# mederrata/spmf

Measured on AMD Instinct MI355X. Metric: elbo_steps_per_sec, higher is better.
Workload: dtype f32

## Files before the change

### spmf_amd/csrc/widek.hip

```cpp
#include "common.h"
#include "kernels.h"

namespace spmf {

namespace {

constexpr int kInFlight = 4;

__device__ __forceinline__ float4 ld4(const float* __restrict__ base, int row, int KP, int sub) {
  return *reinterpret_cast<const float4*>(base + (size_t)row * KP + sub * 4);
}
template <int NH>
__device__ __forceinline__ float group_dot(float4 a, float4 b) {
  if constexpr (NH == 2) {
    const float v = group_sum<16>(dot4(a, b));
    return v + __shfl_xor(v, 16);
  } else {
    return wave_sum(fmaf(a.w, b.w, fmaf(a.z, b.z, fmaf(a.y, b.y, fmaf(a.x, b.x, 0.f)))));
  }
}
template <int NH>
__device__ __forceinline__ float xhalf_add(float v) {
  if constexpr (NH == 2) v += __shfl_xor(v, 32);
  return v;
}
template <int NH>
__device__ __forceinline__ float4 xhalf_add(float4 v) {
  return make_float4(xhalf_add<NH>(v.x), xhalf_add<NH>(v.y), xhalf_add<NH>(v.z), xhalf_add<NH>(v.w));
}

}

template <int KP>
__global__ __launch_bounds__(256) void row_widek_kernel(
    int64_t B, const int32_t* __restrict__ row_ptr, const int32_t* __restrict__ col,
    const float* __restrict__ val, const float* __restrict__ row_scale, const float* __restrict__ Ap,
    const float* __restrict__ Vp, const float* __restrict__ phi, const double* __restrict__ dprep,
    float* __restrict__ z, float* __restrict__ gzs, double* __restrict__ dacc, int mode, int Dcols,
    int64_t dacc_stride) {
  constexpr int NH = 256 / KP, LPG = 64 / NH;
  if (gridDim.y > 1) {
    const size_t sd = blockIdx.y;
    Ap += sd * (size_t)Dcols * KP;
    Vp += sd * (size_t)Dcols * KP;
    phi += sd * (size_t)Dcols;
    dprep += sd * (size_t)kPrepSeg * (KP + 1);
    z += sd * (size_t)B * KP;
    gzs += sd * (size_t)B * KP;
    dacc += sd * (size_t)dacc_stride;
  }
  const bool encode_only = mode == 1;
  const int lane = threadIdx.x & 63, sub = lane % LPG, h = lane / LPG;
  const int64_t wave = ((int64_t)blockIdx.x * blockDim.x + threadIdx.x) >> 6;
  const int64_t nwaves = ((int64_t)gridDim.x * blockDim.x) >> 6;
  float4 veta = make_float4(0.f, 0.f, 0.f, 0.f);
  if (!encode_only)
    veta = make_float4((float)prep_sum(dprep, KP, sub * 4 + 0), (float)prep_sum(dprep, KP, sub * 4 + 1),
                       (float)prep_sum(dprep, KP, sub * 4 + 2), (float)prep_sum(dprep, KP, sub * 4 + 3));
  double ll_acc = 0.0, zsq_acc = 0.0, nnf_acc = 0.0;
  float4 zsum = make_float4(0.f, 0.f, 0.f, 0.f);
  for (int64_t b = wave; b < B; b += nwaves) {
    const int start = row_ptr[b], end = row_ptr[b + 1];
    const float xi = row_scale ? row_scale[b] : 1.f;
    float4 zacc = make_float4(0.f, 0.f, 0.f, 0.f);
    for (int base = start; base < end; base += 64) {
      const int i = base + lane;
      const int c = i < end ? col[i] : 0;
      const float x = i < end ? val[i] : 0.f;
      const int cnt = min(64, end - base);
      for (int e0 = 0; e0 < cnt; e0 += NH * kInFlight) {
        float4 a[kInFlight];
        float xe[kInFlight];
#pragma unroll
        for (int j = 0; j < kInFlight; ++j) {
          const int idx = e0 + NH * j + h, src = min(idx, 63);
          const int cj = __shfl(c, src);
          const float xs = (NH == 2 || idx < cnt) ? __shfl(x, src) : 0.f;
          xe[j] = idx < cnt ? xs : 0.f;
          a[j] = ld4(Ap, cj, KP, sub);
        }
#pragma unroll
        for (int j = 0; j < kInFlight; ++j) zacc = fma4(xe[j], a[j], zacc);
      }
    }
    zacc = xhalf_add<NH>(zacc);
    zacc.x *= xi; zacc.y *= xi; zacc.z *= xi; zacc.w *= xi;
    if (h == 0) reinterpret_cast<float4*>(z + (size_t)b * KP)[sub] = zacc;
    if (encode_only) continue;
    float4 gz = make_float4(0.f, 0.f, 0.f, 0.f);
    float llrow = 0.f;
    for (int base = start; base < end; base += 64) {
      const int i = base + lane;
      const int c = i < end ? col[i] : 0;
      const float x = i < end ? val[i] : 0.f;
      const int cnt = min(64, end - base);
      for (int e0 = 0; e0 < cnt; e0 += NH * kInFlight) {
        float4 vv[kInFlight];
        float xe[kInFlight], ph[kInFlight];
#pragma unroll
        for (int j = 0; j < kInFlight; ++j) {
          const int idx = e0 + NH * j + h, src = min(idx, 63);
          const int cj = __shfl(c, src);
          const float xs = (NH == 2 || idx < cnt) ? __shfl(x, src) : 0.f;
          xe[j] = idx < cnt ? xs : 0.f;
          vv[j] = ld4(Vp, cj, KP, sub);
          ph[j] = phi[cj];
        }
#pragma unroll
        for (int j = 0; j < kInFlight; ++j) {
          const float r = group_dot<NH>(zacc, vv[j]) + ph[j];
          const bool on = xe[j] > 0.f, good = r > 0.f && r < INFINITY;
          const float cc = on ? (good ? xe[j] * __builtin_amdgcn_rcpf(r) : 1.f) : 0.f;
          if (on && good) llrow = fmaf(xe[j], logf(r), llrow);
          if (on && !good) nnf_acc += 1.0;
          gz = fma4(cc, vv[j], gz);
        }
      }
    }
    gz = xhalf_add<NH>(gz);
    if (h == 0) {
      float4 o;
      o.x = xi * (gz.x - veta.x - zacc.x);
      o.y = xi * (gz.y - veta.y - zacc.y);
      o.z = xi * (gz.z - veta.z - zacc.z);
      o.w = xi * (gz.w - veta.w - zacc.w);
      reinterpret_cast<float4*>(gzs + (size_t)b * KP)[sub] = o;
      if constexpr (NH == 2) {
        zsq_acc += (double)dot4(zacc, zacc);
      } else {
        zsq_acc += (double)(zacc.x * zacc.x);
        zsq_acc += (double)(zacc.y * zacc.y);
        zsq_acc += (double)(zacc.z * zacc.z);
        zsq_acc += (double)(zacc.w * zacc.w);
      }
      zsum = add4(zsum, zacc);
    }
    ll_acc += (double)llrow;
  }
  if (encode_only) return;
  dacc += (size_t)(blockIdx.x % kDaccRep) * (kDaccHead + KP);
  const double zq = wave_sum(zsq_acc);
  if (sub == 0) {
    atomicAdd(&dacc[0], ll_acc);
    if (nnf_acc != 0.0) atomicAdd(&dacc[2], nnf_acc);
  }
  if (lane == 0) atomicAdd(&dacc[1], zq);
  if (h == 0) {
    atomicAdd(&dacc[kDaccHead + sub * 4 + 0], (double)zsum.x);
    atomicAdd(&dacc[kDaccHead + sub * 4 + 1], (double)zsum.y);
    atomicAdd(&dacc[kDaccHead + sub * 4 + 2], (double)zsum.z);
    atomicAdd(&dacc[kDaccHead + sub * 4 + 3], (double)zsum.w);
  }
}

template <int KP>
__global__ __launch_bounds__(256) void col_widek_kernel(
    int D, int n_panels, int row_base, int blocks_per_panel, const int32_t* __restrict__ item_ptr,
    const int4* __restrict__ items, const int32_t* __restrict__ pc_row, const float* __restrict__ pc_val,
    const float* __restrict__ Vp, const float* __restrict__ phi, const float* __restrict__ z,
    const float* __restrict__ gzs, float* __restrict__ gAp, float* __restrict__ gVp, float* __restrict__ gphi,
    const int32_t* __restrict__ item_mid, int half_sel, int64_t Brows, int64_t acc_stride,
    const double* __restrict__ pack_dacc, float* __restrict__ pack_tail, int64_t dacc_stride) {
  constexpr int NH = 256 / KP, LPG = 64 / NH;
  if (pack_dacc && blockIdx.x == 0) {
    const double* dacc = pack_dacc + (size_t)blockIdx.y * dacc_stride;
    float* tail = pack_tail + (size_t)blockIdx.y * acc_stride;
    for (int i = threadIdx.x; i < kDaccHead + KP; i += blockDim.x) fold_dacc(i, dacc, tail, KP);
    return;
  }
  if (gridDim.y > 1) {
    const size_t sd = blockIdx.y;
    Vp += sd * (size_t)D * KP;
    phi += sd * (size_t)D;
    z += sd * (size_t)Brows * KP;
    gzs += sd * (size_t)Brows * KP;
    gAp += sd * (size_t)acc_stride;
    gVp += sd * (size_t)acc_stride;
    gphi += sd * (size_t)acc_stride;
  }
  const int lane = threadIdx.x & 63, wid = threadIdx.x >> 6, sub = lane % LPG, h = lane / LPG;
  const int64_t L = (int64_t)blockIdx.x - (pack_dacc ? 1 : 0);
  const int p = (int)(L / blocks_per_panel), ib = (int)(L % blocks_per_panel);
  if (p >= n_panels) return;
  const int ilo = half_sel == 2 ? item_mid[p] : item_ptr[p];
  const int ihi = half_sel == 1 ? item_mid[p] : item_ptr[p + 1];
  const int it = ilo + ib * 4 + wid;
  if (it >= ihi) return;
  const int4 im = items[it];
  const int d = im.z;
  const float4 vp = ld4(Vp, d, KP, sub);
  const float ph = phi[d];
  float4 gV = make_float4(0.f, 0.f, 0.f, 0.f), gA = gV;
  float gph = 0.f;
  const int end = im.x + im.y;
  for (int base = im.x; base < end; base += 64) {
    const int i = base + lane;
    const int rb = i < end ? pc_row[i] - row_base : 0;
    const float x = i < end ? pc_val[i] : 0.f;
    const int cnt = min(64, end - base);
    for (int e0 = 0; e0 < cnt; e0 += NH * kInFlight) {
      float4 zz[kInFlight], gg[kInFlight];
      float xe[kInFlight];
#pragma unroll
      for (int j = 0; j < kInFlight; ++j) {
        const int idx = e0 + NH * j + h, src = min(idx, 63);
        const int b = __shfl(rb, src);
        const float xs = (NH == 2 || idx < cnt) ? __shfl(x, src) : 0.f;
        xe[j] = idx < cnt ? xs : 0.f;
        zz[j] = ld4(z, b, KP, sub);
        gg[j] = ld4(gzs, b, KP, sub);
      }
#pragma unroll
      for (int j = 0; j < kInFlight; ++j) {
        const float r = group_dot<NH>(zz[j], vp) + ph;
        const float xr = (r > 0.f && r < INFINITY) ? xe[j] * __builtin_amdgcn_rcpf(r) : (xe[j] > 0.f ? 1.f : 0.f);
        gV = fma4(xr, zz[j], gV);
        gA = fma4(xe[j], gg[j], gA);
        gph += xr;
      }
    }
  }
  gV = xhalf_add<NH>(gV);
  gA = xhalf_add<NH>(gA);
  gph = xhalf_add<NH>(gph);
  if (h == 0) {
    float* dv = gVp + (size_t)d * KP + sub * 4;
    float* da = gAp + (size_t)d * KP + sub * 4;
    if (gV.x != 0.f) atomicAdd(dv + 0, gV.x);
    if (gV.y != 0.f) atomicAdd(dv + 1, gV.y);
    if (gV.z != 0.f) atomicAdd(dv + 2, gV.z);
    if (gV.w != 0.f) atomicAdd(dv + 3, gV.w);
    if (gA.x != 0.f) atomicAdd(da + 0, gA.x);
    if (gA.y != 0.f) atomicAdd(da + 1, gA.y);
    if (gA.z != 0.f) atomicAdd(da + 2, gA.z);
    if (gA.w != 0.f) atomicAdd(da + 3, gA.w);
    if (lane == 0 && gph != 0.f) atomicAdd(&gphi[d], gph);
  }
}

namespace {
template <int KP>
void row_widek(int nb, const RowArgs& a, hipStream_t st) {
  hipLaunchKernelGGL((row_widek_kernel<KP>), dim3(nb, a.S > 1 ? a.S : 1), dim3(256), 0, st, a.B, a.row_ptr, a.col,
                     a.val, a.row_scale, a.Ap, a.Vp, a.phi, a.dprep, a.z, a.gzs, a.dacc, a.mode, a.D,
                     a.dacc_stride);
}
template <int KP>
void col_widek(int64_t nb, int bpp, const ColArgs& a, hipStream_t st) {
  hipLaunchKernelGGL((col_widek_kernel<KP>), dim3((unsigned)nb, a.S > 1 ? a.S : 1), dim3(256), 0, st, a.D,
                     a.n_panels, a.row_base, bpp, a.item_ptr, reinterpret_cast<const int4*>(a.items), a.pc_row,
                     a.pc_val, a.Vp, a.phi, a.z, a.gzs, a.gAp, a.gVp, a.gphi, a.item_mid, a.half_sel, a.B,
                     a.acc_stride, a.pack_dacc, a.pack_tail, a.dacc_stride);
}
}

bool launch_row_widek(int KP, const RowArgs& a, hipStream_t st) {
  if (a.logt != 0 || (a.mode != 0 && a.mode != 1) || a.det_slots) return false;
  const int64_t want = (a.B + 3) / 4;
  const int nb = (int)(want < 1 ? 1 : (want > 2048 ? 2048 : want));
  return with_kp<256, 128>(KP, [&](auto kp) { row_widek<decltype(kp)::value>(nb, a, st); });
}

bool launch_col_widek(int KP, const ColArgs& a, hipStream_t st) {
  if (a.logt != 0 || a.det_part) return false;
  const int bpp = (a.max_items_per_panel + 3) / 4;
  if (bpp < 1) return false;
  const int64_t nb = (int64_t)a.n_panels * bpp + (a.pack_dacc ? 1 : 0);
  return with_kp<256, 128>(KP, [&](auto kp) { col_widek<decltype(kp)::value>(nb, bpp, a, st); });
}

}
```

Baseline: 379.7.

## Rework wide-K row/col kernels with prefetch, DPP reductions, packed entries, dynamic tail

Rewrites both wide-K kernels. Gather depth grows to groups of 8, and per-entry group dot products are replaced with a three-step DPP/swizzle transpose-fold that reduces eight dots at once. Row pointers and entry chunks are prefetched one and two rows ahead, and a work-stealing dynamic tail balances uneven rows. Optional packed 16+16-bit entries shrink index traffic. The col kernel interleaves panel mapping across blocks and combines halves through LDS before the atomics. This adds complexity and depends on new args (ent, dyn_tail, panel_rows, dyn slot) defined elsewhere. Packed mode truncates values to integers up to 65535.

```diff
diff --git a/spmf_amd/csrc/widek.hip b/spmf_amd/csrc/widek.hip
--- a/spmf_amd/csrc/widek.hip
+++ b/spmf_amd/csrc/widek.hip
@@ -5,40 +5,184 @@
 
 namespace {
 
-constexpr int kInFlight = 4;
+constexpr int kGroup = 8;
+constexpr int kRowBlocks = 2048;
+constexpr int kDynNum = 1, kDynDen = 8;
 
 __device__ __forceinline__ float4 ld4(const float* __restrict__ base, int row, int KP, int sub) {
   return *reinterpret_cast<const float4*>(base + (size_t)row * KP + sub * 4);
 }
+__device__ __forceinline__ float4 zero4() { return make_float4(0.f, 0.f, 0.f, 0.f); }
+
+template <int M>
+__device__ __forceinline__ float lane_xor(float v) {
+  if constexpr (M == 1) {
+    return __int_as_float(__builtin_amdgcn_update_dpp(0, __float_as_int(v), 0xB1, 0xF, 0xF, true));
+  } else if constexpr (M == 2) {
+    return __int_as_float(__builtin_amdgcn_update_dpp(0, __float_as_int(v), 0x4E, 0xF, 0xF, true));
+  } else if constexpr (M < 32) {
+    return __int_as_float(__builtin_amdgcn_ds_swizzle(__float_as_int(v), (M << 10) | 0x1f));
+  } else {
+    return __shfl_xor(v, 32);
+  }
+}
+__host__ __device__ constexpr int fold8_entry(int l) { return ((l & 1) << 2) | (l & 2) | ((l >> 2) & 1); }
+template <int LPG>
+__device__ __forceinline__ float fold8(const float (&p)[kGroup], int lane) {
+  static_assert(kGroup == 8, "three halving steps");
+  const bool b0 = lane & 1, b1 = lane & 2, b2 = lane & 4;
+  float q[4], r[2];
+#pragma unroll
+  for (int i = 0; i < 4; ++i) q[i] = (b0 ? p[i + 4] : p[i]) + lane_xor<1>(b0 ? p[i] : p[i + 4]);
+#pragma unroll
+  for (int i = 0; i < 2; ++i) r[i] = (b1 ? q[i + 2] : q[i]) + lane_xor<2>(b1 ? q[i] : q[i + 2]);
+  float v = (b2 ? r[1] : r[0]) + lane_xor<4>(b2 ? r[0] : r[1]);
+  v += lane_xor<8>(v);
+  v += lane_xor<16>(v);
+  if constexpr (LPG == 64) v += lane_xor<32>(v);
+  return v;
+}
 template <int NH>
-__device__ __forceinline__ float group_dot(float4 a, float4 b) {
+__device__ __forceinline__ int bcast_i(int v, int idx, int h) {
+  const int lo = __builtin_amdgcn_readlane(v, idx);
   if constexpr (NH == 2) {
-    const float v = group_sum<16>(dot4(a, b));
-    return v + __shfl_xor(v, 16);
-  } else {
-    return wave_sum(fmaf(a.w, b.w, fmaf(a.z, b.z, fmaf(a.y, b.y, fmaf(a.x, b.x, 0.f)))));
-  }
+    const int hi = __builtin_amdgcn_readlane(v, idx + 1);
+    return h ? hi : lo;
+  }
+  return lo;
 }
 template <int NH>
-__device__ __forceinline__ float xhalf_add(float v) {
-  if constexpr (NH == 2) v += __shfl_xor(v, 32);
-  return v;
+__device__ __forceinline__ float bcast_f(float v, int idx, int h) {
+  return __int_as_float(bcast_i<NH>(__float_as_int(v), idx, h));
+}
+template <int NH>
+__device__ __forceinline__ float owner_bcast(float w, int j, int h) {
+  const int lo = __builtin_amdgcn_readlane(__float_as_int(w), fold8_entry(j));
+  if constexpr (NH == 2) {
+    const int hi = __builtin_amdgcn_readlane(__float_as_int(w), 32 + fold8_entry(j));
+    return __int_as_float(h ? hi : lo);
+  }
+  return __int_as_float(lo);
 }
 template <int NH>
 __device__ __forceinline__ float4 xhalf_add(float4 v) {
-  return make_float4(xhalf_add<NH>(v.x), xhalf_add<NH>(v.y), xhalf_add<NH>(v.z), xhalf_add<NH>(v.w));
-}
-
-}
-
-template <int KP>
+  if constexpr (NH == 2) {
+    v.x += __shfl_xor(v.x, 32); v.y += __shfl_xor(v.y, 32);
+    v.z += __shfl_xor(v.z, 32); v.w += __shfl_xor(v.w, 32);
+  }
+  return v;
+}
+
+template <bool PACKED>
+__device__ __forceinline__ void ld_entry(const int32_t* __restrict__ idx, const float* __restrict__ val,
+                                         const uint32_t* __restrict__ ent, int i, bool ok, int& ra, float& rb) {
+  if constexpr (PACKED) {
+    ra = ok ? (int)ent[i] : 0;
+    rb = 0.f;
+  } else {
+    ra = ok ? idx[i] : 0;
+    rb = ok ? val[i] : 0.f;
+  }
+}
+template <bool PACKED>
+__device__ __forceinline__ void entry_of(int ra, float rb, int& c, float& x) {
+  if constexpr (PACKED) {
+    c = (int)((uint32_t)ra >> 16);
+    x = (float)((uint32_t)ra & 0xffffu);
+  } else {
+    c = ra;
+    x = rb;
+  }
+}
+
+template <int KP, bool FULL>
+__device__ __forceinline__ void row_s1_group(const float* __restrict__ Ap, int c, float x, int e0, int cnt, int sub,
+                                             int h, float4& zacc) {
+  constexpr int NH = 256 / KP;
+  float4 a[kGroup];
+  float xe[kGroup];
+#pragma unroll
+  for (int j = 0; j < kGroup; ++j) {
+    const int i0 = e0 + NH * j;
+    const int cj = bcast_i<NH>(c, i0, h);
+    xe[j] = bcast_f<NH>(x, i0, h);
+    a[j] = (FULL || i0 + h < cnt) ? ld4(Ap, cj, KP, sub) : zero4();
+  }
+#pragma unroll
+  for (int j = 0; j < kGroup; ++j) zacc = fma4(xe[j], a[j], zacc);
+}
+template <int KP, bool FULL>
+__device__ __forceinline__ void row_s2_group(const float* __restrict__ Vp, const float* __restrict__ phi, int c,
+                                             float x, int e0, int cnt, int lane, int sub, int h, const float4& z,
+                                             float4& gz, float& ll, double& nnf) {
+  constexpr int NH = 256 / KP, LPG = 64 / NH;
+  float4 vv[kGroup];
+#pragma unroll
+  for (int j = 0; j < kGroup; ++j) {
+    const int i0 = e0 + NH * j;
+    const int cj = bcast_i<NH>(c, i0, h);
+    vv[j] = (FULL || i0 + h < cnt) ? ld4(Vp, cj, KP, sub) : zero4();
+  }
+  const int mine = e0 + NH * fold8_entry(lane & 7) + h;
+  const int cs = __shfl(c, mine);
+  const float xs = __shfl(x, mine);
+  const float ph = phi[cs];
+  float p[kGroup];
+#pragma unroll
+  for (int j = 0; j < kGroup; ++j) p[j] = dot4(z, vv[j]);
+  const float r = fold8<LPG>(p, lane) + ph;
+  const bool on = mine < cnt && xs > 0.f, good = r > 0.f && r < INFINITY;
+  const float cc = on ? (good ? xs * __builtin_amdgcn_rcpf(r) : 1.f) : 0.f;
+  if (sub < 8) {
+    ll = fmaf(on && good ? xs : 0.f, logf(good ? r : 1.f), ll);
+    if (on && !good) nnf += 1.0;
+  }
+#pragma unroll
+  for (int j = 0; j < kGroup; ++j) gz = fma4(owner_bcast<NH>(cc, j, h), vv[j], gz);
+}
+
+template <int KP, bool FULL>
+__device__ __forceinline__ void col_group(const float* __restrict__ z, const float* __restrict__ gzs, int rb, float x,
+                                          int e0, int cnt, int lane, int sub, int h, const float4& vp, float ph,
+                                          float4& gV, float4& gA, float& gph) {
+  constexpr int NH = 256 / KP, LPG = 64 / NH;
+  float4 zz[kGroup], gg[kGroup];
+  float xe[kGroup];
+#pragma unroll
+  for (int j = 0; j < kGroup; ++j) {
+    const int i0 = e0 + NH * j;
+    const int b = bcast_i<NH>(rb, i0, h);
+    xe[j] = bcast_f<NH>(x, i0, h);
+    const bool ld = FULL || i0 + h < cnt;
+    zz[j] = ld ? ld4(z, b, KP, sub) : zero4();
+    gg[j] = ld ? ld4(gzs, b, KP, sub) : zero4();
+  }
+  const int mine = e0 + NH * fold8_entry(lane & 7) + h;
+  const float xs = __shfl(x, mine);
+  float p[kGroup];
+#pragma unroll
+  for (int j = 0; j < kGroup; ++j) p[j] = dot4(zz[j], vp);
+  const float r = fold8<LPG>(p, lane) + ph;
+  const float xr = (r > 0.f && r < INFINITY) ? xs * __builtin_amdgcn_rcpf(r) : (xs > 0.f ? 1.f : 0.f);
+  if (sub < 8) gph += xr;
+#pragma unroll
+  for (int j = 0; j < kGroup; ++j) {
+    gV = fma4(owner_bcast<NH>(xr, j, h), zz[j], gV);
+    gA = fma4(xe[j], gg[j], gA);
+  }
+}
+
+}
+
+template <int KP, bool PACKED>
 __global__ __launch_bounds__(256) void row_widek_kernel(
     int64_t B, const int32_t* __restrict__ row_ptr, const int32_t* __restrict__ col,
-    const float* __restrict__ val, const float* __restrict__ row_scale, const float* __restrict__ Ap,
-    const float* __restrict__ Vp, const float* __restrict__ phi, const double* __restrict__ dprep,
-    float* __restrict__ z, float* __restrict__ gzs, double* __restrict__ dacc, int mode, int Dcols,
-    int64_t dacc_stride) {
+    const float* __restrict__ val, const uint32_t* __restrict__ ent, const float* __restrict__ row_scale,
+    const float* __restrict__ Ap, const float* __restrict__ Vp, const float* __restrict__ phi,
+    const double* __restrict__ dprep, float* __restrict__ z, float* __restrict__ gzs, double* __restrict__ dacc,
+    int mode, int Dcols, int64_t dacc_stride, int dyn_tail) {
   constexpr int NH = 256 / KP, LPG = 64 / NH;
+  constexpr int EG = NH * kGroup;
   if (gridDim.y > 1) {
     const size_t sd = blockIdx.y;
     Ap += sd * (size_t)Dcols * KP;
@@ -51,100 +195,148 @@
   }
   const bool encode_only = mode == 1;
   const int lane = threadIdx.x & 63, sub = lane % LPG, h = lane / LPG;
-  const int64_t wave = ((int64_t)blockIdx.x * blockDim.x + threadIdx.x) >> 6;
+  const int64_t wave = (int64_t)blockIdx.x * (blockDim.x >> 6) +
+                       __builtin_amdgcn_readfirstlane((int)(threadIdx.x >> 6));
   const int64_t nwaves = ((int64_t)gridDim.x * blockDim.x) >> 6;
-  float4 veta = make_float4(0.f, 0.f, 0.f, 0.f);
+  float4 veta = zero4();
   if (!encode_only)
     veta = make_float4((float)prep_sum(dprep, KP, sub * 4 + 0), (float)prep_sum(dprep, KP, sub * 4 + 1),
                        (float)prep_sum(dprep, KP, sub * 4 + 2), (float)prep_sum(dprep, KP, sub * 4 + 3));
   double ll_acc = 0.0, zsq_acc = 0.0, nnf_acc = 0.0;
-  float4 zsum = make_float4(0.f, 0.f, 0.f, 0.f);
-  for (int64_t b = wave; b < B; b += nwaves) {
-    const int start = row_ptr[b], end = row_ptr[b + 1];
-    const float xi = row_scale ? row_scale[b] : 1.f;
-    float4 zacc = make_float4(0.f, 0.f, 0.f, 0.f);
-    for (int base = start; base < end; base += 64) {
-      const int i = base + lane;
-      const int c = i < end ? col[i] : 0;
-      const float x = i < end ? val[i] : 0.f;
-      const int cnt = min(64, end - base);
-      for (int e0 = 0; e0 < cnt; e0 += NH * kInFlight) {
-        float4 a[kInFlight];
-        float xe[kInFlight];
-#pragma unroll
-        for (int j = 0; j < kInFlight; ++j) {
-          const int idx = e0 + NH * j + h, src = min(idx, 63);
-          const int cj = __shfl(c, src);
-          const float xs = (NH == 2 || idx < cnt) ? __shfl(x, src) : 0.f;
-          xe[j] = idx < cnt ? xs : 0.f;
-          a[j] = ld4(Ap, cj, KP, sub);
-        }
-#pragma unroll
-        for (int j = 0; j < kInFlight; ++j) zacc = fma4(xe[j], a[j], zacc);
+  float4 zsum = zero4();
+
+  int64_t B_static = B, dyn_lo = B, dyn_hi = B;
+  unsigned int* dyn_ctr = nullptr;
+  if (dyn_tail && !encode_only) {
+    const int64_t per_wave = B / nwaves;
+    if (per_wave >= 8) {
+      int64_t fixed = per_wave - (per_wave * kDynNum) / kDynDen;
+      if (fixed < 2) fixed = 2;
+      B_static = fixed * nwaves;
+      const int r = (int)(wave & (kDaccRep - 1));
+      const int64_t each = (B - B_static + kDaccRep - 1) / kDaccRep;
+      dyn_lo = B_static + r * each;
+      dyn_hi = dyn_lo + each < B ? dyn_lo + each : B;
+      if (dyn_lo > B) dyn_lo = B;
+      dyn_ctr = reinterpret_cast<unsigned int*>(dacc + (size_t)r * (kDaccHead + KP) + kDaccDynSlot);
+    }
+  }
+  auto fixed_next = [&](int64_t cur) -> int64_t {
+    if (cur >= B) return B;
+    if (cur + nwaves < B_static) return cur + nwaves;
+    return dyn_ctr ? (int64_t)-1 : B;
+  };
+  auto take_dynamic = [&]() -> int64_t {
+    unsigned int k = 0;
+    if (lane == 0) k = atomicAdd(dyn_ctr, 1u);
+    k = (unsigned int)__builtin_amdgcn_readfirstlane((int)k);
+    const int64_t row = dyn_lo + (int64_t)k;
+    return row < dyn_hi ? row : B;
+  };
+  auto ptr_of = [&](int64_t row, int& s, int& e, float& sc) {
+    s = __builtin_amdgcn_readfirstlane(row_ptr[row]);
+    e = __builtin_amdgcn_readfirstlane(row_ptr[row + 1]);
+    sc = row_scale ? row_scale[row] : 1.f;
+  };
+
+  int start = 0, end = 0, pc = 0, nstart = 0, nend = 0;
+  float xi = 1.f, px = 0.f, nxi = 1.f;
+  int64_t b = wave < B_static ? wave : B;
+  int64_t bn = fixed_next(b);
+  if (bn < 0) bn = take_dynamic();
+  int64_t bnn = fixed_next(bn);
+  if (bnn < 0) bnn = take_dynamic();
+  if (b < B) {
+    ptr_of(b, start, end, xi);
+    ld_entry<PACKED>(col, val, ent, start + lane, start + lane < end, pc, px);
+  }
+  if (bn < B) ptr_of(bn, nstart, nend, nxi);
+  while (b < B) {
+    int qc = 0, nnstart = 0, nnend = 0;
+    float qx = 0.f, nnxi = 1.f;
+    if (bn < B) ld_entry<PACKED>(col, val, ent, nstart + lane, nstart + lane < nend, qc, qx);
+    if (bnn < B) ptr_of(bnn, nnstart, nnend, nnxi);
+    int64_t bnnn = fixed_next(bnn);
+    unsigned int dyn_k = 0;
+    const bool dyn_ask = bnnn < 0;
+    if (dyn_ask && lane == 0) dyn_k = atomicAdd(dyn_ctr, 1u);
+    float4 zacc = zero4();
+    {
+      int ra = pc;
+      float rb = px;
+      for (int base = start; base < end; base += 64) {
+        int ra2;
+        float rb2;
+        const int i2 = base + 64 + lane;
+        ld_entry<PACKED>(col, val, ent, i2, i2 < end, ra2, rb2);
+        int c;
+        float x;
+        entry_of<PACKED>(ra, rb, c, x);
+        const int cnt = min(64, end - base);
+        int e0 = 0;
+        for (; e0 + EG <= cnt; e0 += EG) row_s1_group<KP, true>(Ap, c, x, e0, cnt, sub, h, zacc);
+        if (e0 < cnt) row_s1_group<KP, false>(Ap, c, x, e0, cnt, sub, h, zacc);
+        ra = ra2;
+        rb = rb2;
       }
     }
     zacc = xhalf_add<NH>(zacc);
     zacc.x *= xi; zacc.y *= xi; zacc.z *= xi; zacc.w *= xi;
     if (h == 0) reinterpret_cast<float4*>(z + (size_t)b * KP)[sub] = zacc;
-    if (encode_only) continue;
-    float4 gz = make_float4(0.f, 0.f, 0.f, 0.f);
+    float4 gz = zero4();
     float llrow = 0.f;
-    for (int base = start; base < end; base += 64) {
-      const int i = base + lane;
-      const int c = i < end ? col[i] : 0;
-      const float x = i < end ? val[i] : 0.f;
-      const int cnt = min(64, end - base);
-      for (int e0 = 0; e0 < cnt; e0 += NH * kInFlight) {
-        float4 vv[kInFlight];
-        float xe[kInFlight], ph[kInFlight];
-#pragma unroll
-        for (int j = 0; j < kInFlight; ++j) {
-          const int idx = e0 + NH * j + h, src = min(idx, 63);
-          const int cj = __shfl(c, src);
-          const float xs = (NH == 2 || idx < cnt) ? __shfl(x, src) : 0.f;
-          xe[j] = idx < cnt ? xs : 0.f;
-          vv[j] = ld4(Vp, cj, KP, sub);
-          ph[j] = phi[cj];
-        }
-#pragma unroll
-        for (int j = 0; j < kInFlight; ++j) {
-          const float r = group_dot<NH>(zacc, vv[j]) + ph[j];
-          const bool on = xe[j] > 0.f, good = r > 0.f && r < INFINITY;
-          const float cc = on ? (good ? xe[j] * __builtin_amdgcn_rcpf(r) : 1.f) : 0.f;
-          if (on && good) llrow = fmaf(xe[j], logf(r), llrow);
-          if (on && !good) nnf_acc += 1.0;
-          gz = fma4(cc, vv[j], gz);
-        }
+    if (!encode_only) {
+      int ra = pc;
+      float rb = px;
+      for (int base = start; base < end; base += 64) {
+        int ra2;
+        float rb2;
+        const int i2 = base + 64 + lane;
+        ld_entry<PACKED>(col, val, ent, i2, i2 < end, ra2, rb2);
+        int c;
+        float x;
+        entry_of<PACKED>(ra, rb, c, x);
+        const int cnt = min(64, end - base);
+        int e0 = 0;
+        for (; e0 + EG <= cnt; e0 += EG)
+          row_s2_group<KP, true>(Vp, phi, c, x, e0, cnt, lane, sub, h, zacc, gz, llrow, nnf_acc);
+        if (e0 < cnt) row_s2_group<KP, false>(Vp, phi, c, x, e0, cnt, lane, sub, h, zacc, gz, llrow, nnf_acc);
+        ra = ra2;
+        rb = rb2;
       }
     }
+    const float xi_cur = xi;
+    const int64_t b_cur = b;
+    start = nstart; end = nend; xi = nxi;
+    pc = qc; px = qx;
+    nstart = nnstart; nend = nnend; nxi = nnxi;
+    if (dyn_ask) {
+      const int64_t row = dyn_lo + (int64_t)(unsigned int)__builtin_amdgcn_readfirstlane((int)dyn_k);
+      bnnn = row < dyn_hi ? row : B;
+    }
+    b = bn; bn = bnn; bnn = bnnn;
+    if (encode_only) continue;
     gz = xhalf_add<NH>(gz);
     if (h == 0) {
       float4 o;
-      o.x = xi * (gz.x - veta.x - zacc.x);
-      o.y = xi * (gz.y - veta.y - zacc.y);
-      o.z = xi * (gz.z - veta.z - zacc.z);
-      o.w = xi * (gz.w - veta.w - zacc.w);
-      reinterpret_cast<float4*>(gzs + (size_t)b * KP)[sub] = o;
-      if constexpr (NH == 2) {
-        zsq_acc += (double)dot4(zacc, zacc);
-      } else {
-        zsq_acc += (double)(zacc.x * zacc.x);
-        zsq_acc += (double)(zacc.y * zacc.y);
-        zsq_acc += (double)(zacc.z * zacc.z);
-        zsq_acc += (double)(zacc.w * zacc.w);
-      }
+      o.x = xi_cur * (gz.x - veta.x - zacc.x);
+      o.y = xi_cur * (gz.y - veta.y - zacc.y);
+      o.z = xi_cur * (gz.z - veta.z - zacc.z);
+      o.w = xi_cur * (gz.w - veta.w - zacc.w);
+      reinterpret_cast<float4*>(gzs + (size_t)b_cur * KP)[sub] = o;
+      zsq_acc += (double)dot4(zacc, zacc);
       zsum = add4(zsum, zacc);
     }
     ll_acc += (double)llrow;
   }
   if (encode_only) return;
   dacc += (size_t)(blockIdx.x % kDaccRep) * (kDaccHead + KP);
-  const double zq = wave_sum(zsq_acc);
-  if (sub == 0) {
-    atomicAdd(&dacc[0], ll_acc);
-    if (nnf_acc != 0.0) atomicAdd(&dacc[2], nnf_acc);
-  }
-  if (lane == 0) atomicAdd(&dacc[1], zq);
+  const double llw = wave_sum(ll_acc), zq = wave_sum(zsq_acc), nfw = wave_sum(nnf_acc);
+  if (lane == 0) {
+    atomicAdd(&dacc[0], llw);
+    atomicAdd(&dacc[1], zq);
+    if (nfw != 0.0) atomicAdd(&dacc[2], nfw);
+  }
   if (h == 0) {
     atomicAdd(&dacc[kDaccHead + sub * 4 + 0], (double)zsum.x);
     atomicAdd(&dacc[kDaccHead + sub * 4 + 1], (double)zsum.y);
@@ -153,15 +345,15 @@
   }
 }
 
-template <int KP>
+template <int KP, bool PACKED>
 __global__ __launch_bounds__(256) void col_widek_kernel(
     int D, int n_panels, int row_base, int blocks_per_panel, const int32_t* __restrict__ item_ptr,
     const int4* __restrict__ items, const int32_t* __restrict__ pc_row, const float* __restrict__ pc_val,
-    const float* __restrict__ Vp, const float* __restrict__ phi, const float* __restrict__ z,
-    const float* __restrict__ gzs, float* __restrict__ gAp, float* __restrict__ gVp, float* __restrict__ gphi,
-    const int32_t* __restrict__ item_mid, int half_sel, int64_t Brows, int64_t acc_stride,
+    const uint32_t* __restrict__ pc_ent, int panel_rows, const float* __restrict__ Vp, const float* __restrict__ phi,
+    const float* __restrict__ z, const float* __restrict__ gzs, float* __restrict__ gAp, float* __restrict__ gVp,
+    float* __restrict__ gphi, const int32_t* __restrict__ item_mid, int half_sel, int64_t Brows, int64_t acc_stride,
     const double* __restrict__ pack_dacc, float* __restrict__ pack_tail, int64_t dacc_stride) {
-  constexpr int NH = 256 / KP, LPG = 64 / NH;
+  constexpr int NH = 256 / KP, LPG = 64 / NH, EG = NH * kGroup;
   if (pack_dacc && blockIdx.x == 0) {
     const double* dacc = pack_dacc + (size_t)blockIdx.y * dacc_stride;
     float* tail = pack_tail + (size_t)blockIdx.y * acc_stride;
@@ -178,95 +370,107 @@
     gVp += sd * (size_t)acc_stride;
     gphi += sd * (size_t)acc_stride;
   }
-  const int lane = threadIdx.x & 63, wid = threadIdx.x >> 6, sub = lane % LPG, h = lane / LPG;
+  __shared__ __attribute__((aligned(16))) float stage[4][NH][2 * KP];
+  const int lane = threadIdx.x & 63, sub = lane % LPG, h = lane / LPG;
+  const int wid = __builtin_amdgcn_readfirstlane((int)(threadIdx.x >> 6));
   const int64_t L = (int64_t)blockIdx.x - (pack_dacc ? 1 : 0);
-  const int p = (int)(L / blocks_per_panel), ib = (int)(L % blocks_per_panel);
+  int p, ib;
+  if (n_panels < 8) {
+    p = (int)(L / blocks_per_panel);
+    ib = (int)(L % blocks_per_panel);
+  } else {
+    const int64_t q = L >> 3;
+    p = 8 * (int)(q / blocks_per_panel) + (int)(L & 7);
+    ib = (int)(q % blocks_per_panel);
+  }
   if (p >= n_panels) return;
   const int ilo = half_sel == 2 ? item_mid[p] : item_ptr[p];
   const int ihi = half_sel == 1 ? item_mid[p] : item_ptr[p + 1];
   const int it = ilo + ib * 4 + wid;
   if (it >= ihi) return;
   const int4 im = items[it];
-  const int d = im.z;
+  const int first = __builtin_amdgcn_readfirstlane(im.x);
+  const int end = first + __builtin_amdgcn_readfirstlane(im.y);
+  const int d = __builtin_amdgcn_readfirstlane(im.z);
+  int ra;
+  float rv;
+  ld_entry<PACKED>(pc_row, pc_val, pc_ent, first + lane, first + lane < end, ra, rv);
   const float4 vp = ld4(Vp, d, KP, sub);
   const float ph = phi[d];
-  float4 gV = make_float4(0.f, 0.f, 0.f, 0.f), gA = gV;
+  const int pbase = PACKED ? p * panel_rows : -row_base;
+  float4 gV = zero4(), gA = zero4();
   float gph = 0.f;
-  const int end = im.x + im.y;
-  for (int base = im.x; base < end; base += 64) {
-    const int i = base + lane;
-    const int rb = i < end ? pc_row[i] - row_base : 0;
-    const float x = i < end ? pc_val[i] : 0.f;
+  for (int base = first; base < end; base += 64) {
+    int ra2;
+    float rv2;
+    const int i2 = base + 64 + lane;
+    ld_entry<PACKED>(pc_row, pc_val, pc_ent, i2, i2 < end, ra2, rv2);
+    int rb;
+    float x;
+    entry_of<PACKED>(ra, rv, rb, x);
+    rb = base + lane < end ? rb + pbase : 0;
     const int cnt = min(64, end - base);
-    for (int e0 = 0; e0 < cnt; e0 += NH * kInFlight) {
-      float4 zz[kInFlight], gg[kInFlight];
-      float xe[kInFlight];
-#pragma unroll
-      for (int j = 0; j < kInFlight; ++j) {
-        const int idx = e0 + NH * j + h, src = min(idx, 63);
-        const int b = __shfl(rb, src);
-        const float xs = (NH == 2 || idx < cnt) ? __shfl(x, src) : 0.f;
-        xe[j] = idx < cnt ? xs : 0.f;
-        zz[j] = ld4(z, b, KP, sub);
-        gg[j] = ld4(gzs, b, KP, sub);
-      }
-#pragma unroll
-      for (int j = 0; j < kInFlight; ++j) {
-        const float r = group_dot<NH>(zz[j], vp) + ph;
-        const float xr = (r > 0.f && r < INFINITY) ? xe[j] * __builtin_amdgcn_rcpf(r) : (xe[j] > 0.f ? 1.f : 0.f);
-        gV = fma4(xr, zz[j], gV);
-        gA = fma4(xe[j], gg[j], gA);
-        gph += xr;
-      }
-    }
-  }
-  gV = xhalf_add<NH>(gV);
-  gA = xhalf_add<NH>(gA);
-  gph = xhalf_add<NH>(gph);
-  if (h == 0) {
-    float* dv = gVp + (size_t)d * KP + sub * 4;
-    float* da = gAp + (size_t)d * KP + sub * 4;
-    if (gV.x != 0.f) atomicAdd(dv + 0, gV.x);
-    if (gV.y != 0.f) atomicAdd(dv + 1, gV.y);
-    if (gV.z != 0.f) atomicAdd(dv + 2, gV.z);
-    if (gV.w != 0.f) atomicAdd(dv + 3, gV.w);
-    if (gA.x != 0.f) atomicAdd(da + 0, gA.x);
-    if (gA.y != 0.f) atomicAdd(da + 1, gA.y);
-    if (gA.z != 0.f) atomicAdd(da + 2, gA.z);
-    if (gA.w != 0.f) atomicAdd(da + 3, gA.w);
-    if (lane == 0 && gph != 0.f) atomicAdd(&gphi[d], gph);
-  }
+    int e0 = 0;
+    for (; e0 + EG <= cnt; e0 += EG) col_group<KP, true>(z, gzs, rb, x, e0, cnt, lane, sub, h, vp, ph, gV, gA, gph);
+    if (e0 < cnt) col_group<KP, false>(z, gzs, rb, x, e0, cnt, lane, sub, h, vp, ph, gV, gA, gph);
+    ra = ra2;
+    rv = rv2;
+  }
+  float4* st4 = reinterpret_cast<float4*>(&stage[wid][h][0]);
+  st4[sub] = gV;
+  st4[KP / 4 + sub] = gA;
+  gph = wave_sum(gph);
+  __builtin_amdgcn_wave_barrier();
+#pragma unroll
+  for (int i = 0; i < (2 * KP) / 64; ++i) {
+    const int e = i * 64 + lane;
+    float v = stage[wid][0][e];
+    if constexpr (NH == 2) v += stage[wid][1][e];
+    float* dst = i * 64 < KP ? gVp + (size_t)d * KP + e : gAp + (size_t)d * KP + (e - KP);
+    if (v != 0.f) atomicAdd(dst, v);
+  }
+  if (lane == 0 && gph != 0.f) atomicAdd(&gphi[d], gph);
 }
 
 namespace {
-template <int KP>
+template <int KP, bool PACKED>
 void row_widek(int nb, const RowArgs& a, hipStream_t st) {
-  hipLaunchKernelGGL((row_widek_kernel<KP>), dim3(nb, a.S > 1 ? a.S : 1), dim3(256), 0, st, a.B, a.row_ptr, a.col,
-                     a.val, a.row_scale, a.Ap, a.Vp, a.phi, a.dprep, a.z, a.gzs, a.dacc, a.mode, a.D,
-                     a.dacc_stride);
-}
-template <int KP>
+  hipLaunchKernelGGL((row_widek_kernel<KP, PACKED>), dim3(nb, a.S > 1 ? a.S : 1), dim3(256), 0, st, a.B, a.row_ptr,
+                     a.col, a.val, a.ent, a.row_scale, a.Ap, a.Vp, a.phi, a.dprep, a.z, a.gzs, a.dacc, a.mode, a.D,
+                     a.dacc_stride, a.dyn_tail);
+}
+template <int KP, bool PACKED>
 void col_widek(int64_t nb, int bpp, const ColArgs& a, hipStream_t st) {
-  hipLaunchKernelGGL((col_widek_kernel<KP>), dim3((unsigned)nb, a.S > 1 ? a.S : 1), dim3(256), 0, st, a.D,
+  hipLaunchKernelGGL((col_widek_kernel<KP, PACKED>), dim3((unsigned)nb, a.S > 1 ? a.S : 1), dim3(256), 0, st, a.D,
                      a.n_panels, a.row_base, bpp, a.item_ptr, reinterpret_cast<const int4*>(a.items), a.pc_row,
-                     a.pc_val, a.Vp, a.phi, a.z, a.gzs, a.gAp, a.gVp, a.gphi, a.item_mid, a.half_sel, a.B,
-                     a.acc_stride, a.pack_dacc, a.pack_tail, a.dacc_stride);
+                     a.pc_val, a.pc_ent, a.panel_rows, a.Vp, a.phi, a.z, a.gzs, a.gAp, a.gVp, a.gphi, a.item_mid,
+                     a.half_sel, a.B, a.acc_stride, a.pack_dacc, a.pack_tail, a.dacc_stride);
 }
 }
 
 bool launch_row_widek(int KP, const RowArgs& a, hipStream_t st) {
   if (a.logt != 0 || (a.mode != 0 && a.mode != 1) || a.det_slots) return false;
   const int64_t want = (a.B + 3) / 4;
-  const int nb = (int)(want < 1 ? 1 : (want > 2048 ? 2048 : want));
-  return with_kp<256, 128>(KP, [&](auto kp) { row_widek<decltype(kp)::value>(nb, a, st); });
+  const int nb = (int)(want < 1 ? 1 : (want > kRowBlocks ? kRowBlocks : want));
+  return with_kp<256, 128>(KP, [&](auto kp) {
+    constexpr int K = decltype(kp)::value;
+    if (a.ent) row_widek<K, true>(nb, a, st);
+    else row_widek<K, false>(nb, a, st);
+  });
 }
 
 bool launch_col_widek(int KP, const ColArgs& a, hipStream_t st) {
   if (a.logt != 0 || a.det_part) return false;
   const int bpp = (a.max_items_per_panel + 3) / 4;
   if (bpp < 1) return false;
-  const int64_t nb = (int64_t)a.n_panels * bpp + (a.pack_dacc ? 1 : 0);
-  return with_kp<256, 128>(KP, [&](auto kp) { col_widek<decltype(kp)::value>(nb, bpp, a, st); });
-}
-
-}
+  const int64_t nt = (a.n_panels + 7) / 8;
+  const int64_t nb = (a.n_panels < 8 ? (int64_t)a.n_panels * bpp : nt * bpp * 8) + (a.pack_dacc ? 1 : 0);
+  const bool packed = a.pc_ent && a.panel_rows > 0 && a.panel_rows <= 65536;
+  return with_kp<256, 128>(KP, [&](auto kp) {
+    constexpr int K = decltype(kp)::value;
+    if (packed) col_widek<K, true>(nb, bpp, a, st);
+    else col_widek<K, false>(nb, bpp, a, st);
+  });
+}
+
+}
```

Measured after the change: 378.7. About the same (-0.3%).
